# Francis-Rings/MotionEditor

Hardware: AMD Instinct MI355X
Metric: denoise-steps/sec, 24f x 512^2 two-branch UNet3D+ControlNet(+adapter+K/V injection) (higher is better)
Workload: dtype f16

## Files before the change

include/motioned.h:

```cpp
#ifndef MOTIONED_H
#define MOTIONED_H

#include <stdint.h>

#ifdef __cplusplus
extern "C" {
#endif

#define ME_OK 0
#define ME_EINVAL (-1)
#define ME_EHIP (-2)

#define ME_ABI_VERSION 9

int me_abi_version(void);
const char* me_last_error(void);
const char* me_last_kernel(void);
int me_device_info(int* cus, int* lds_bytes, char* arch, int arch_len);

#define ME_GATHER_DENSE 0
#define ME_GATHER_CONV3 1
#define ME_GATHER_TCONV 2

typedef struct me_gemm_args {
// ... 10 lines not shown
  const void* bias;
  const void* rowvec;
  int32_t ldrv, rows_per_vec;
  const void* res;
  int32_t ldr;
  const void* res2;
  int32_t ldr2;
  int32_t geglu;
  int32_t act;
  float alpha;
  int32_t res_rows;
  int32_t res2_rows;
  void* work;
  int64_t work_bytes;
  int32_t splits_;
  int32_t sel_rows;
  void* C2;
  int32_t c2_col0, c2_dh;
  int64_t c2_hs;
  int32_t m_off;
  const void* ln_stats;
  const void* ln_colsum;
  const void* ln_cvec;
  int64_t ln_stride;
  int32_t ln_parts;
  float ln_eps;
  void* ln_out;
  int64_t ln_out_stride;
} me_gemm_args;

int me_gemm(const me_gemm_args* a, void* stream);
int me_ln_stats(const void* X, int32_t ldx, int64_t rows, int32_t C, void* stats, int64_t stride, void* stream);
int64_t me_gemm_work_bytes(const me_gemm_args* a);

typedef struct me_conv_small_args {
  const void* in;
  const void* W;
  const void* bias;
  void* out;
  int32_t n_img, Cin, Cout, H, Wd;
  int64_t img_stride, ch_stride;
  int32_t in_is_f16;
  int32_t silu;
  int32_t frames;
  int64_t frame_stride;
} me_conv_small_args;

int me_conv_small(const me_conv_small_args* a, void* stream);

#define ME_SEG_PLAIN 0
#define ME_SEG_DUAL_CUR 1
#define ME_SEG_DUAL_PREV 2
#define ME_SEG_DUAL_BIN 3

typedef struct me_attn_args {
  const void* Q;
  const void* K;
  const void* V;
  void* O;
  int32_t ldq, ldk, ldv, ldo;
  int32_t heads, dh;
  int32_t n_items, nq, nk, nseg;
  const int32_t* seg_item;
  const int32_t* seg_mode;
  const void* mask;
  float scale;
// ... 199 lines not shown
```

motioneditor_amd/capi.py:

```python
from __future__ import annotations

import ctypes as C
from pathlib import Path

LIB_PATH = Path(__import__("os").environ.get("ME_LIB") or Path(__file__).resolve().parent / "libmotioned.so")

ME_OK, ME_EINVAL, ME_EHIP = 0, -1, -2
ABI_VERSION = 9
GATHER_DENSE, GATHER_CONV3, GATHER_TCONV = 0, 1, 2
SEG_PLAIN, SEG_DUAL_CUR, SEG_DUAL_PREV, SEG_DUAL_BIN = 0, 1, 2, 3

_i32, _i64, _f32, _vp = C.c_int32, C.c_int64, C.c_float, C.c_void_p


class GemmArgs(C.Structure):
    _fields_ = [
        ("X", _vp), ("W", _vp), ("C", _vp),
        ("M", _i32), ("N", _i32), ("K", _i32),
        ("ldx", _i32), ("ldc", _i32), ("gather", _i32),
        ("Hin", _i32), ("Win", _i32), ("Hout", _i32), ("Wout", _i32), ("stride", _i32), ("ups", _i32), ("pad0", _i32),
        ("frames", _i32), ("npix", _i32), ("chunk", _i32),
        ("frame0", _i32), ("frames_total", _i32), ("halo_prev", _i32), ("halo_next", _i32),
        ("bias", _vp), ("rowvec", _vp), ("ldrv", _i32), ("rows_per_vec", _i32),
        ("res", _vp), ("ldr", _i32), ("res2", _vp), ("ldr2", _i32), ("geglu", _i32), ("act", _i32), ("alpha", _f32), ("res_rows", _i32), ("res2_rows", _i32),
# ... 60 lines not shown
        ("q_frames", _i32), ("q_frame0", _i32), ("kv_parts", _i32), ("q_parts", _i32),
    ]


class GroupNormArgs(C.Structure):
    _fields_ = [
        ("X", _vp), ("Y", _vp), ("gamma", _vp), ("beta", _vp), ("stats", _vp),
        ("rows", _i32), ("rows_per_group", _i32),
        ("C", _i32), ("ldx", _i32), ("ldy", _i32), ("groups", _i32), ("eps", _f32), ("silu", _i32),
    ]


class LayerNormArgs(C.Structure):
    _fields_ = [
        ("X", _vp), ("Y", _vp), ("gamma", _vp), ("beta", _vp),
        ("rows", _i32), ("C", _i32), ("ldx", _i32), ("ldy", _i32), ("eps", _f32),
    ]


class PlanStats(C.Structure):
    _fields_ = [("launches", _i64), ("event_records", _i64), ("event_waits", _i64), ("arg_bytes", _i64), ("replays", _i64), ("streams", _i32)]


class PlanNodeInfo(C.Structure):
    _fields_ = [("kind", _i32), ("stream", _i32), ("event", _i32), ("grid", C.c_uint32 * 3), ("block", C.c_uint32 * 3), ("lds_bytes", C.c_uint32),
                ("n_args", _i32), ("arg_bytes", _i64)]


PLAN_LAUNCH, PLAN_RECORD, PLAN_WAIT = 0, 1, 2

SYMBOLS = {
    "me_abi_version": (C.c_int, []),
    "me_gemm_work_bytes": (_i64, [C.POINTER(GemmArgs)]),
    "me_last_error": (C.c_char_p, []),
    "me_last_kernel": (C.c_char_p, []),
    "me_device_info": (C.c_int, [C.POINTER(C.c_int), C.POINTER(C.c_int), C.c_char_p, C.c_int]),
    "me_gemm": (C.c_int, [C.POINTER(GemmArgs), _vp]),
    "me_conv_small": (C.c_int, [C.POINTER(ConvSmallArgs), _vp]),
    "me_attn": (C.c_int, [C.POINTER(AttnArgs), _vp]),
    "me_tattn": (C.c_int, [C.POINTER(TAttnArgs), _vp]),
    "me_groupnorm": (C.c_int, [C.POINTER(GroupNormArgs), _vp]),
    "me_groupnorm_scratch_bytes": (C.c_int64, [_i32, _i32, _i32]),
    "me_groupnorm_stats": (C.c_int, [C.POINTER(GroupNormArgs), _vp]),
    "me_groupnorm_apply": (C.c_int, [C.POINTER(GroupNormArgs), _i64, _vp]),
    "me_layernorm": (C.c_int, [C.POINTER(LayerNormArgs), _vp]),
    "me_ln_stats": (C.c_int, [_vp, _i32, _i64, _i32, _vp, _i64, _vp]),
    "me_softmax_rows": (C.c_int, [_vp, _i32, _vp, _i32, _i64, _i32, _vp]),
    "me_axpy_rows": (C.c_int, [_vp, _i32, _vp, _i32, _vp, _i32, _i64, _i32, _f32, _vp]),
    "me_attn_vsum_bytes": (_i64, [_i32, _i32]),
    "me_attn_fallback_blocks": (_i64, [_i32]),
    "me_geglu_bwd": (C.c_int, [_vp, _i32, _vp, _i32, _vp, _i32, _i64, _i32, _vp]),
    "me_layernorm_bwd": (C.c_int, [_vp, _i32, _vp, _i32, _vp, _vp, _i32, _i64, _i32, C.c_float, _vp]),
    "me_groupnorm_bwd": (C.c_int, [_vp, _i32, _vp, _i32, _vp, _vp, _vp, _i32, _i64, _i32, _i32, _i32, C.c_float, _i32, _vp, _vp]),
    "me_groupnorm_bwd_scratch_bytes": (_i64, [_i32, _i32, _i32]),
    "me_tattn_bwd": (C.c_int, [_vp, _i32, _vp, _i32, _vp, _i32, _vp, _i32, _vp, _i32, _vp, _i32, _vp, _i32, _i32, _i32, _i32, _i32, _i32, C.c_float, _vp]),
    "me_softmax_bwd_rows": (C.c_int, [_vp, _i32, _vp, _i32, _vp, _i32, _i64, _i32, C.c_float, _vp]),
    "me_relu_bwd": (C.c_int, [_vp, _i32, _vp, _i32, _vp, _i32, _i64, _i32, _vp]),
    "me_copy_rows": (C.c_int, [_vp, _i32, _vp, _i32, _i64, _i32, _vp]),
    "me_copy_blocks": (C.c_int, [_vp, _i32, _vp, _i32, _i32, _i32, _i64, _i32, _i64, _i64, _i64, _i64, _vp]),
    "me_silu": (C.c_int, [_vp, _vp, _i64, _vp]),
    "me_relu": (C.c_int, [_vp, _vp, _i64, _vp]),
    "me_timestep_embed": (C.c_int, [_vp, _i32, _i32, _f32, _vp]),
    "me_cfg_ddim": (C.c_int, [_vp, _vp, _vp, _i32, _i32, _i32, _i32, _i32, _f32, _f32, _f32, _vp]),
    "me_timestep_embed_dev": (C.c_int, [_vp, _i32, _i32, _vp, _vp]),
    "me_cfg_ddim_dev": (C.c_int, [_vp, _vp, _vp, _i32, _i32, _i32, _i32, _i32, _vp, _vp]),
    "me_gaussian_sample": (C.c_int, [_vp, _vp, _i32, _vp, _i32, _i32, _f32, _vp]),
# ... 69 lines not shown
```

motioneditor_amd/csrc/gemm.hip:

```cpp
#include "me_common.h"
#include "../../include/motioned.h"
#include <stdio.h>
#include <stdlib.h>

namespace {

constexpr int BK = 64;
#ifndef WIDE_TERMS
#define WIDE_TERMS 0
#endif
constexpr int STAGE_REG = 0, STAGE_GLDS = 1, STAGE_BUF = 2;
constexpr int ROWEPI_FLAG = 1 << 30, TILEORDER_FLAG = 1 << 29;

template <bool NT = false>
__device__ __forceinline__ void st16(f16* p, uint4 v) {
  if constexpr (NT) {
    typedef unsigned u32x4 __attribute__((ext_vector_type(4)));
    __builtin_nontemporal_store((u32x4){v.x, v.y, v.z, v.w}, reinterpret_cast<u32x4*>(p));
  } else {
    *reinterpret_cast<uint4*>(p) = v;
  }
}
template <bool NT = false>
__device__ __forceinline__ void st8(f16* p, uint2 v) {
// ... 43 lines not shown
    const int ky = tap / 3, kx = tap - ky * 3;
    const int iy = r.y0 + ky, ix = r.x0 + kx;
    const int sh = a.ups ? 1 : 0;
    const int Hv = a.Hin << sh, Wv = a.Win << sh;
    if (iy < 0 || iy >= Hv || ix < 0 || ix >= Wv) return -1;
    if (a.ups == 2 && ((iy | ix) & 1)) return -1;
    return r.base + (iy >> sh) * a.Win + (ix >> sh);
  }
  const int dt = tap - 1;
  const int ftot = a.frames_total > 0 ? a.frames_total : a.frames;
  const int gf = a.frame0 + r.y0, gs = gf + dt;
  if (gs < 0 || gs >= ftot || gs / a.chunk != gf / a.chunk) return -1;
  const int ls = r.y0 + dt;
  if (ls >= 0 && ls < a.frames) return r.base + dt * a.npix;
  const int hb = ls < 0 ? a.halo_prev : a.halo_next;
  return hb < 0 ? -1 : hb + r.x0;
}

template <int NT, int MT, int WN>
__device__ __forceinline__ void init_acc(const me_gemm_args& a, f32x4 (&acc)[NT][MT], int n0, int wn, int lane, bool use_bias = true) {
  const f16* __restrict__ bias = use_bias ? reinterpret_cast<const f16*>(a.bias) : nullptr;
  const int nb = n0 + wn * WN + (lane >> 4) * 4;
  const float inv_alpha = bias ? 1.0f / a.alpha : 0.f;
#pragma unroll
  for (int j = 0; j < NT; ++j) {
    U64 b;
    b.u = (bias && nb + 16 * j < a.N) ? *reinterpret_cast<const uint2*>(bias + nb + 16 * j) : make_uint2(0u, 0u);
    const f32x4 v = {(float)b.e[0] * inv_alpha, (float)b.e[1] * inv_alpha, (float)b.e[2] * inv_alpha, (float)b.e[3] * inv_alpha};
#pragma unroll
    for (int i = 0; i < MT; ++i) acc[j][i] = v;
  }
}

template <int NT, int MT>
__device__ __forceinline__ void ln_fold_acc(const me_gemm_args& a, f32x4 (&acc)[NT][MT], int mbase, int nbase, int lane) {
  const float* __restrict__ st = reinterpret_cast<const float*>(a.ln_stats);
  const float* __restrict__ cs = reinterpret_cast<const float*>(a.ln_colsum);
  const float* __restrict__ cv = reinterpret_cast<const float*>(a.ln_cvec);
  const float invK = 1.0f / (float)a.K;
  float nmean[MT], rstd[MT];
#pragma unroll
  for (int i = 0; i < MT; ++i) {
    const int m = min(mbase + i * 16 + (lane & 15), a.M - 1);
    float s1 = 0.f, s2 = 0.f;
    for (int p = 0; p < a.ln_parts; ++p) {
      const f32x2 v = *reinterpret_cast<const f32x2*>(st + (long)p * a.ln_stride + 2 * (long)m);
      s1 += v[0];
      s2 += v[1];
    }
    const float mu = s1 * invK;
    const float var = __builtin_fmaf(-mu, mu, s2 * invK);
    nmean[i] = -mu;
    rstd[i] = rsqrtf(fmaxf(var, 0.f) + a.ln_eps);
  }
#pragma unroll
  for (int j = 0; j < NT; ++j) {
    const int n = nbase + j * 16 + (lane >> 4) * 4;
    f32x4 s = {0.f, 0.f, 0.f, 0.f}, c = {0.f, 0.f, 0.f, 0.f};
    if (n < a.N) {
      s = *reinterpret_cast<const f32x4*>(cs + n);
      c = *reinterpret_cast<const f32x4*>(cv + n);
    }
#pragma unroll
    for (int i = 0; i < MT; ++i)
#pragma unroll
      for (int r = 0; r < 4; ++r) acc[j][i][r] = __builtin_fmaf(rstd[i], __builtin_fmaf(nmean[i], s[r], acc[j][i][r]), c[r]);
  }
}

constexpr int LN_LDS_BYTES = 12288, LN_LDS_COLSUM = 8192, LN_LDS_CVEC = 10240;
template <int NT, int MT>
__device__ __forceinline__ void ln_fold_acc_lds(const me_gemm_args& a, f32x4 (&acc)[NT][MT], const char* img, int rloc, int cloc, int lane) {
  const float invK = 1.0f / (float)a.K;
  uint2 v[MT][4];
#pragma unroll
  for (int i = 0; i < MT; ++i) {
    const int row = rloc + i * 16 + (lane & 15);
#pragma unroll
    for (int p = 0; p < 4; ++p) v[i][p] = *reinterpret_cast<const uint2*>(img + p * 2048 + row * 8);
  }
  float nmean[MT], rstd[MT];
#pragma unroll
  for (int i = 0; i < MT; ++i) {
    float s1 = 0.f, s2 = 0.f;
#pragma unroll
    for (int p = 0; p < 4; ++p) {
      s1 += __uint_as_float(v[i][p].x);
      s2 += __uint_as_float(v[i][p].y);
    }
    const float mu = s1 * invK;
    const float var = __builtin_fmaf(-mu, mu, s2 * invK);
    nmean[i] = -mu;
    rstd[i] = rsqrtf(fmaxf(var, 0.f) + a.ln_eps);
  }
#pragma unroll
  for (int j = 0; j < NT; ++j) {
    const int col = cloc + j * 16 + (lane >> 4) * 4;
    const uint4 su = *reinterpret_cast<const uint4*>(img + LN_LDS_COLSUM + col * 4), cu = *reinterpret_cast<const uint4*>(img + LN_LDS_CVEC + col * 4);
    const f32x4 s = {__uint_as_float(su.x), __uint_as_float(su.y), __uint_as_float(su.z), __uint_as_float(su.w)};
    const f32x4 c = {__uint_as_float(cu.x), __uint_as_float(cu.y), __uint_as_float(cu.z), __uint_as_float(cu.w)};
// ... 1103 lines not shown
    cluster(1, 0, NT0);
    ME_BAR();
  }
  if (wr == 0) ME_BAR();
  asm volatile("s_waitcnt vmcnt(0)" ::: "memory");
#undef ME_BAR
#undef ME_LGKM0

  if constexpr (EPI <= 0) {
    if (a.ln_stats) {
      if constexpr (LN_LDS) ln_fold_acc_lds<NT, MT>(a, acc, smem + 2 * BUFBYTES, wr * GR, wc * WN, lane);
      else ln_fold_acc<NT, MT>(a, acc, m0 + wr * GR, n0 + wc * WN, lane);
    }
  }

  if constexpr (EPI >= 0 && BN == 256) {
    __builtin_amdgcn_s_barrier();
    return epilogue_geglu_rowpass<NT, MT, WN>(a, acc, m0, n0, wr, wc, lane, smem);
  } else if constexpr (EPI >= 0) {
    __builtin_amdgcn_s_barrier();
    char* scr = smem + wave * (32 * (WN * 2 + 16));
    const int mw0 = m0 + wr * GR, nw0 = n0 + wc * WN;
    const LnOutCtx lnx = {m0, wr, wc, tid, smem + 8 * (32 * (WN * 2 + 16))};
    return epilogue_rowpass<EPI, NT, MT, WN>(a, acc, mw0, nw0, lane, scr, lnx);
  } else {
    auto rowfn = [&](int i) {
      const int m = m0 + wr * GR + i * 16 + (lane & 15);
      return m < a.M ? m : -1;
    };
    epilogue<NT, MT, WN>(a, acc, rowfn, m0, n0, wc, lane, nullptr, 0);
  }
}

__global__ __launch_bounds__(256) void gemm_splitk_reduce_kernel(const me_gemm_args a) {
  const int vpr = a.N / 4;
  const long total = (long)a.M * vpr;
  const float* __restrict__ wk = reinterpret_cast<const float*>(a.work);
  const f16* __restrict__ bias = reinterpret_cast<const f16*>(a.bias);
  const f16* __restrict__ rowvec = reinterpret_cast<const f16*>(a.rowvec);
  const f16* res = reinterpret_cast<const f16*>(a.res);
  const f16* res2 = reinterpret_cast<const f16*>(a.res2);
  f16* C = reinterpret_cast<f16*>(a.C);
  const long plane = (long)a.M * a.N;
  for (long idx = (long)blockIdx.x * 256 + threadIdx.x; idx < total; idx += (long)gridDim.x * 256) {
    const int m = (int)(idx / vpr);
    const int n = (int)(idx - (long)m * vpr) * 4;
    f32x4 v = *reinterpret_cast<const f32x4*>(wk + (long)m * a.N + n);
    for (int s_ = 1; s_ < a.splits_; ++s_) v += *reinterpret_cast<const f32x4*>(wk + s_ * plane + (long)m * a.N + n);
    v *= a.alpha;
    if (bias) {
      U64 b;
      b.u = *reinterpret_cast<const uint2*>(bias + n);
#pragma unroll
      for (int r = 0; r < 4; ++r) v[r] += (float)b.e[r];
    }
    U64 rv, r1, r2, o;
    if (rowvec) rv.u = *reinterpret_cast<const uint2*>(rowvec + (long)(m / a.rows_per_vec) * a.ldrv + n);
    if (res) r1.u = *reinterpret_cast<const uint2*>(res + (long)(a.res_rows > 0 ? m % a.res_rows : m) * a.ldr + n);
    if (res2) r2.u = *reinterpret_cast<const uint2*>(res2 + (long)(a.res2_rows > 0 ? m % a.res2_rows : m) * a.ldr2 + n);
    if (a.act == 0) {
#pragma unroll
      for (int r = 0; r < 4; ++r) {
        f16 h = (f16)v[r];
        if (rowvec) h = h + rv.e[r];
        if (res) h = h + r1.e[r];
        if (res2) h = h + r2.e[r];
// ... 271 lines not shown
  const int nit = (a->K / 64) * (a->gather == ME_GATHER_CONV3 ? 9 : (a->gather == ME_GATHER_TCONV ? 3 : 1));
  const long blocks = (long)((a->M + 127) / 128) * ((a->N + 159) / 160);
  const int S = choose_split(a, blocks, nit);
  return S > 1 ? (int64_t)4 * a->M * a->N * 4 : 0;
}

static int gemm_dispatch(const me_gemm_args* a, void* stream);

extern "C" int me_gemm(const me_gemm_args* a, void* stream) {
  if (!a || !a->X || !a->W || !a->C) { me_set_error("me_gemm: null pointer"); return ME_EINVAL; }
  if (a->ln_stats) {
    if (a->gather != ME_GATHER_DENSE || a->bias || a->alpha != 1.0f || a->rowvec || a->res || a->res2 || a->act || !a->ln_colsum || !a->ln_cvec || a->ln_parts < 1 || a->ln_parts > 4 || a->ln_stride < 2 * (int64_t)a->M ||
        (a->ln_stride & 1) || ((uintptr_t)a->ln_stats & 7) || (((uintptr_t)a->ln_colsum | (uintptr_t)a->ln_cvec) & 15) || !(a->ln_eps > 0.f)) {
      me_set_error("me_gemm: a LayerNorm-folded launch is dense, has no bias (it is inside ln_cvec), no rowvec / residual / activation and alpha == 1; ln_colsum / ln_cvec fp32 [N] 16-byte aligned, "
                   "ln_stats 8-byte aligned with 1 <= ln_parts <= 4 parts ln_stride >= 2 M floats apart, ln_eps > 0");
      return ME_EINVAL;
    }
  }
  if (a->ln_out && (a->geglu || a->C2 || a->N % 8 || a->N > 1536 || a->ldc % 8 || ((uintptr_t)a->C & 15) || ((uintptr_t)a->ln_out & 7) || a->ln_out_stride < 2 * (int64_t)a->M || (a->ln_out_stride & 1))) {
    me_set_error("me_gemm: ln_out needs a plain fp16 output of N % 8 == 0, N <= 1536 columns (no GEGLU, no head-major panels), ldc % 8 == 0, and parts >= 2 M floats apart");
    return ME_EINVAL;
  }
  g_ln_fused = false;
  const int rc = gemm_dispatch(a, stream);
  if (rc != ME_OK || !a->ln_out || g_ln_fused) return rc;
  char nm[96];
  snprintf(nm, sizeof(nm), "%s", me_last_kernel());
  const int rc2 = me_ln_stats(reinterpret_cast<const f16*>(a->C) + (long)a->m_off * a->ldc, a->ldc, (int64_t)a->M - a->m_off, a->N,
                              reinterpret_cast<float*>(a->ln_out) + 2 * (long)a->m_off, a->ln_out_stride, stream);
  me_set_kernel(nm);
  return rc2;
}

static int gemm_dispatch(const me_gemm_args* a, void* stream) {
  if (a->M <= 0 || a->N <= 0 || a->K <= 0) { me_set_error("me_gemm: non-positive dimension"); return ME_EINVAL; }
  if (a->K % 8 || a->ldx % 8 || a->ldc % 4 || a->N % 4) { me_set_error("me_gemm: K, ldx must be multiples of 8 and N, ldc of 4"); return ME_EINVAL; }
  if (((uintptr_t)a->X | (uintptr_t)a->W) & 15 || ((uintptr_t)a->C & 7)) { me_set_error("me_gemm: misaligned pointer"); return ME_EINVAL; }
  if (a->gather < 0 || a->gather > 2) { me_set_error("me_gemm: bad gather mode"); return ME_EINVAL; }
  if (a->gather == ME_GATHER_CONV3) {
    if (a->Hin <= 0 || a->Win <= 0 || a->Hout <= 0 || a->Wout <= 0 || (a->stride != 1 && a->stride != 2) || a->ups < 0 || a->ups > 2 ||
        (a->pad0 != 0 && a->pad0 != 1) || a->M % (a->Hout * a->Wout)) { me_set_error("me_gemm: bad conv geometry"); return ME_EINVAL; }
  }
  if (a->gather == ME_GATHER_TCONV) {
    const int ftot = a->frames_total > 0 ? a->frames_total : a->frames;
    if (a->frames <= 0 || a->npix <= 0 || a->chunk <= 0 || ftot % a->chunk || (a->m_off == 0 && a->sel_rows <= a->M && a->M % (a->frames * a->npix)) || a->frame0 < 0 ||
        a->frame0 + a->frames > ftot) { me_set_error("me_gemm: bad tconv geometry"); return ME_EINVAL; }
  }
  if (a->rowvec && (a->rows_per_vec <= 0 || a->ldrv % 4 || ((uintptr_t)a->rowvec & 7))) { me_set_error("me_gemm: bad rowvec"); return ME_EINVAL; }
  if (a->res && (a->ldr % 4 || ((uintptr_t)a->res & 7))) { me_set_error("me_gemm: bad residual"); return ME_EINVAL; }
  if (a->res2 && (a->ldr2 % 4 || ((uintptr_t)a->res2 & 7))) { me_set_error("me_gemm: bad second residual"); return ME_EINVAL; }
  if (a->res_rows < 0 || a->res2_rows < 0) { me_set_error("me_gemm: negative res_rows"); return ME_EINVAL; }
  if (a->act < 0 || a->act > 2) { me_set_error("me_gemm: bad activation"); return ME_EINVAL; }
  if (a->bias && ((uintptr_t)a->bias & 7)) { me_set_error("me_gemm: misaligned bias"); return ME_EINVAL; }
  if (a->geglu && (a->N % 32 || a->rowvec || a->res || a->res2 || a->act || a->alpha != 1.0f)) { me_set_error("me_gemm: geglu needs N % 32 == 0, alpha == 1 and no rowvec/res/act"); return ME_EINVAL; }
  if (a->m_off < 0 || a->m_off >= a->M || (a->m_off > 0 && a->gather == ME_GATHER_CONV3)) { me_set_error("me_gemm: m_off must lie in [0, M) and is for dense / TemporalConv launches"); return ME_EINVAL; }
  if (a->C2 && (a->geglu || a->act || a->rowvec || a->res || a->res2 || a->c2_dh <= 0 || a->c2_dh % 8 || a->c2_col0 < 0 || a->c2_col0 % 16 || a->c2_col0 >= a->N ||
                (a->N - a->c2_col0) % a->c2_dh || a->c2_hs % 8 || a->c2_hs < (int64_t)a->M * a->c2_dh || ((uintptr_t)a->C2 & 15) || a->gather == ME_GATHER_CONV3)) {
    me_set_error("me_gemm: head-major output (C2) needs a term-free epilogue, c2_dh % 8 == 0, c2_col0 % 16 == 0, whole heads, c2_hs % 8 == 0 and >= M * c2_dh, 16-byte alignment");
    return ME_EINVAL;
  }
  hipStream_t st = reinterpret_cast<hipStream_t>(stream);
  const bool wide = a->N % 128 == 0 || a->N % 64 != 0;
  if (stage_impl() == STAGE_GLDS) {
    const int Msel = a->sel_rows > a->M ? a->sel_rows : a->M;
    const long big_blocks = (long)((Msel + 255) / 256) * (a->N / 320);
    if (a->gather == ME_GATHER_CONV3 && a->stride == 1 && a->ups == 0 && !a->pad0 && a->N % 320 == 0 && a->K % 64 == 0 && a->Hin % 16 == 0 &&
// ... 31 lines not shown
```

motioneditor_amd/models/graph.py:

```python
from __future__ import annotations

import contextlib
from dataclasses import dataclass
from typing import Callable, List, Optional, Sequence

import torch

from .. import ops, plan, segments
from ..weights import Packed

HEADS = 8
ADAPTER_CHUNK = 8
HEAD_MAJOR_Q = __import__("os").environ.get("ME_HEAD_MAJOR_Q", "1") != "0"
HEAD_MAJOR_KV = __import__("os").environ.get("ME_HEAD_MAJOR_KV", "1") != "0"
SPLIT_SHARDED_TCONV = __import__("os").environ.get("ME_SPLIT_TCONV", "1") != "0"
INPLACE_SKIPS = __import__("os").environ.get("ME_INPLACE_SKIPS", "1") != "0"
LN_FOLD = __import__("os").environ.get("ME_LN_FOLD", "1") != "0"
COND_EMBED_CACHE = True


@dataclass
class Act:
    t: torch.Tensor
    B: int
    f: int
    h: int
    w: int
    cat: Optional[torch.Tensor] = None

    @property
    def N(self) -> int:
        return self.h * self.w

    @property
    def C(self) -> int:
        return self.t.shape[1]

    def like(self, t: torch.Tensor, h: Optional[int] = None, w: Optional[int] = None) -> "Act":
        return Act(t, self.B, self.f, self.h if h is None else h, self.w if w is None else w)

    def rows_of(self, b: int) -> torch.Tensor:
        n = self.f * self.N
        return self.t[b * n:(b + 1) * n]


@dataclass
class AttnCall:
    q: torch.Tensor
    k: torch.Tensor
    v: torch.Tensor
# ... 81 lines not shown
    return LN_FOLD and not getattr(ops, "recording", False) and getattr(ops, "LN_FOLD", False)


def _gemm_st(*args, **kw):
    if _fold():
        return ops.gemm(*args, ln_out=True, **kw)
    return ops.gemm(*args, **kw), None


class LN:

    def __init__(self, P: Packed, norm: str, x: torch.Tensor, stats: Optional[torch.Tensor] = None):
        self.P, self.norm, self.x, self.stats, self._rows = P, norm, x, stats, None

    def rows(self) -> torch.Tensor:
        if self._rows is None:
            self._rows = ops.layernorm(self.x, self.P.vec(self.norm + ".weight"), self.P.vec(self.norm + ".bias"))
        return self._rows

    def gemm(self, names: Sequence[str], *, geglu_bias: Optional[str] = None, **kw):
        names = list(names)
        geglu = geglu_bias is not None
        if _fold() and self._rows is None:
            if self.stats is None:
                self.stats = ops.ln_stats(self.x)
            w, cs, cv = self.P.ln_fold(self.norm, names, geglu=geglu, bias=geglu_bias)
            return ops.gemm(self.x, w, ln=(self.stats, cs, cv, 1e-5), geglu=geglu, **kw)
        if geglu:
            return ops.gemm(self.rows(), self.P.geglu_mat(names[0]), bias=self.P.geglu_vec(geglu_bias), geglu=True, **kw)
        return ops.gemm(self.rows(), self.P.fused(names) if len(names) > 1 else self.P.mat(names[0]), **kw)


def feed_forward(P: Packed, p: str, n: "LN", res: torch.Tensor, want_stats: bool = False):
    g = n.gemm([p + ".net.0.proj.weight"], geglu_bias=p + ".net.0.proj.bias")
    return (_gemm_st if want_stats else (lambda *a, **k: (ops.gemm(*a, **k), None)))(g, P.mat(p + ".net.2.weight"), bias=P.vec(p + ".net.2.bias"), res=res)


def _ln(P: Packed, p: str, x: torch.Tensor) -> torch.Tensor:
    return ops.layernorm(x, P.vec(p + ".weight"), P.vec(p + ".bias"))


def _qkv(P: Packed, p: str, n: "LN", C: int, shard, B: int = 0, N: int = 0, head_major: bool = False):
    names = [p + ".to_q.weight", p + ".to_k.weight", p + ".to_v.weight"]
    if shard is None:
        if head_major and HEAD_MAJOR_KV and not getattr(ops, "recording", False) and getattr(ops, "HEAD_MAJOR_KV", False):
            if HEAD_MAJOR_Q:
                _, qkv = n.gemm(names, head_major=(0, C // HEADS))
                return qkv[:HEADS], qkv[HEADS:2 * HEADS], qkv[2 * HEADS:]
            q, kv = n.gemm(names, head_major=(C, C // HEADS))
            return q, kv[:HEADS], kv[HEADS:]
        qkv = n.gemm(names)
        return qkv[:, :C], qkv[:, C:2 * C], qkv[:, 2 * C:]
    ext, loc = shard.kv_buffer(n.x.shape[0], 2 * C, B, N, n.x)
    n.gemm(names[1:], out=loc)
    pending = shard.start_kv(ext, B, N, ops.copy_rows)
    q = n.gemm(names[:1])
    kv = shard.finish_kv(pending)
    return q, kv[:, :C], kv[:, C:]


def _temporal_attn(P: Packed, p: str, n: "LN", C: int, B: int, f: int, N: int, dh: int, shard, editor=None, place: str = "") -> torch.Tensor:
    def go(tc):
        return editor(call=tc, is_cross=False, place_in_unet=place, num_heads=HEADS) if editor is not None else tc.run()
    if shard is not None and shard.pixel_sharded(N):
        r = shard.to_pixel_shards(n.rows(), B * f, N, ops.copy_blocks)
        qkv = ops.gemm(r, P.fused([p + ".to_q.weight", p + ".to_k.weight", p + ".to_v.weight"]))
# ... 462 lines not shown
```

motioneditor_amd/ops.py:

```python
from __future__ import annotations

import ctypes as C
from typing import Optional, Sequence, Tuple

import os

import torch

from . import capi
from .capi import AttnArgs, AttnBwdArgs, ConvSmallArgs, GemmArgs, GemmDwArgs, GroupNormArgs, LayerNormArgs, TAttnArgs

F16 = torch.float16


_raw_stream = getattr(torch._C, "_cuda_getCurrentRawStream", None)
_cur_device = getattr(torch._C, "_cuda_getDevice", None)


def _stream() -> int:
    if _raw_stream is not None and _cur_device is not None:
        return _raw_stream(_cur_device())
    return torch.cuda.current_stream().cuda_stream


# ... 83 lines not shown
        if col0 == 0:
            out = panels.view(-1)[:8 * M].view(M, 8)
    if out is None:
        if row_range is not None:
            raise ValueError("gemm: row_range writes into a caller-provided `out` of all M rows")
        out = empty(M, n_out, x)
    _chk2d(out, "gemm.out")
    if out.shape[0] < M or out.shape[1] < n_out:
        raise ValueError("gemm: out too small")
    a.X, a.W, a.C = x.data_ptr(), w.data_ptr(), out.data_ptr()
    a.M, a.N, a.K = M, N, K
    if row_range is not None:
        lo, hi = row_range
        if not (0 <= lo < hi <= M) or conv is not None:
            raise ValueError("gemm: row_range must lie inside [0, M) (dense / TemporalConv launches)")
        a.m_off, a.M = lo, hi
        a.sel_rows = max(a.sel_rows, M)
    a.ldx, a.ldc = x.stride(0), out.stride(0)
    a.bias = _p(bias)
    if rowvec is not None:
        _chk2d(rowvec, "gemm.rowvec")
        a.rowvec, a.ldrv, a.rows_per_vec = rowvec.data_ptr(), rowvec.stride(0), rows_per_vec
    if res is not None:
        _chk2d(res, "gemm.res")
        a.res, a.ldr = res.data_ptr(), res.stride(0)
    if res2 is not None:
        _chk2d(res2, "gemm.res2")
        a.res2, a.ldr2 = res2.data_ptr(), res2.stride(0)
    a.geglu = 1 if geglu else 0
    a.act = act
    a.alpha = alpha
    a.res_rows, a.res2_rows = res_rows, res2_rows
    if ln is not None:
        st_, cs_, cv_, eps_ = ln
        if st_.dtype != torch.float32 or st_.dim() != 3 or st_.shape[2] != 2 or st_.stride(2) != 1 or st_.stride(1) != 2 or st_.shape[1] < M \
                or cs_.dtype != torch.float32 or cv_.dtype != torch.float32 or cs_.numel() != N or cv_.numel() != N or not cs_.is_contiguous() or not cv_.is_contiguous():
            raise ValueError("gemm: ln = (fp32 stats [parts, rows, 2], fp32 colsum [N], fp32 cvec [N], eps)")
        a.ln_stats, a.ln_colsum, a.ln_cvec, a.ln_eps = st_.data_ptr(), cs_.data_ptr(), cv_.data_ptr(), eps_
        a.ln_parts, a.ln_stride = st_.shape[0], st_.stride(0)
    so = None
    if ln_out:
        if panels is not None or geglu:
            raise ValueError("gemm: ln_out is for plain row outputs")
        so = torch.empty((n_out // 320 if n_out % 320 == 0 else 1, M, 2), dtype=torch.float32, device=x.device)
        a.ln_out, a.ln_out_stride = so.data_ptr(), so.stride(0)
    if SELECT_ROWS_SCALE > 1:
        a.sel_rows = M * SELECT_ROWS_SCALE
    for r_, n_ in ((res, res_rows), (res2, res2_rows)):
        if r_ is not None and r_.shape[0] < (n_ or M):
            raise ValueError("gemm: residual has fewer rows than the output reads")
    if N >= 1280 and M <= 8192:
        nb = capi.lib().me_gemm_work_bytes(C.byref(a))
        if nb > 0:
            a.work, a.work_bytes = _work(nb, x.device, "splitk").data_ptr(), nb
    e0 = _pb()
    capi.check(capi.lib().me_gemm(C.byref(a), _stream()), "me_gemm")
    if e0 is not None:
        rows_in = (M // (conv[2] * conv[3])) * conv[0] * conv[1] if conv is not None else M
        n_terms = (res is not None) + (res2 is not None)
        n_hm = panels.numel() // M if panels is not None else 0
        _pe(e0, "gemm", 2.0 * M * N * K * taps, 2.0 * (rows_in * K + N * K * taps + M * n_out * (1 + n_terms) + M * n_hm), f"M{M} N{N} K{K} taps{taps}{' geglu' if geglu else ''}{' +b' if bias is not None else ''}{' +rv' if rowvec is not None else ''}"
            f"{' +res' if res is not None else ''}{' +res2' if res2 is not None else ''}{' act' + str(act) if act else ''}{' a' + str(alpha) if alpha != 1.0 else ''}{' ln' if ln is not None else ''}{' lnout' if ln_out else ''}", _last_kernel())
    if panels is not None and n_out == 0:
        return None, panels
    out = out[:M, :n_out] if (out.shape[0] != M or out.shape[1] != n_out) else out
    if so is not None:
        return out, so
    return out if panels is None else (out, panels)


def ln_stats(x: torch.Tensor) -> torch.Tensor:
    _chk2d(x, "ln_stats.x")
    rows, Cc = x.shape
    st = torch.empty((Cc // 320 if Cc % 320 == 0 else 1, rows, 2), dtype=torch.float32, device=x.device)
    e0 = _pb()
    capi.check(capi.lib().me_ln_stats(x.data_ptr(), x.stride(0), rows, Cc, st.data_ptr(), st.stride(0), _stream()), "me_ln_stats")
    _pe(e0, "layernorm", 3.0 * rows * Cc, 2.0 * rows * Cc, "stats", "ln_stats")
    return st


def gemm_splits_k(M: int, N: int, K: int, taps: int = 1) -> bool:
    if not (N >= 1280 and M <= 8192):
        return False
    a = GemmArgs()
    a.M, a.N, a.K = M, N, K
    a.gather = capi.GATHER_TCONV if taps == 3 else (capi.GATHER_CONV3 if taps == 9 else capi.GATHER_DENSE)
    return capi.lib().me_gemm_work_bytes(C.byref(a)) > 0


def conv_small(inp: torch.Tensor, w: torch.Tensor, bias: Optional[torch.Tensor], *, n_img: int, Cin: int, H: int, Wd: int,
               img_stride: int, ch_stride: int, frames: int = 0, frame_stride: int = 0, silu: bool = False) -> torch.Tensor:
    if w.dtype != torch.float32 or (bias is not None and bias.dtype != torch.float32):
        raise ValueError("conv_small: weights and bias must be fp32")
    Cout = w.shape[0]
    out = torch.empty((n_img * H * Wd, Cout), dtype=F16, device=inp.device)
    a = ConvSmallArgs()
    a.inp, a.W, a.bias, a.out = inp.data_ptr(), w.data_ptr(), _p(bias), out.data_ptr()
    a.n_img, a.Cin, a.Cout, a.H, a.Wd = n_img, Cin, Cout, H, Wd
    a.img_stride, a.ch_stride = img_stride, ch_stride
    if inp.dtype == torch.float32:
        a.in_is_f16 = 0
# ... 601 lines not shown
```

Before: 6.733.

## Fuse LayerNorm-folded GEGLU FF1 and FF2 into one FFN kernel for C=320

Adds an ffn_kernel that, for each 128-row block, computes the LN-folded GEGLU projection in 128-column hidden slices. Each slice is kept in LDS and immediately multiplied into the FF2 accumulator with bias, residual and optional LN-stats epilogue. This avoids writing and re-reading the M x 1280 hidden activation to global memory and drops one launch per feed-forward at width 320. In exchange it uses one 512-thread block per CU with large LDS and streams weights repeatedly per block, so grid parallelism and weight traffic change.

```diff
diff --git a/include/motioned.h b/include/motioned.h
--- a/include/motioned.h
+++ b/include/motioned.h
@@ -66,6 +66,7 @@
 int me_gemm(const me_gemm_args* a, void* stream);
 int me_ln_stats(const void* X, int32_t ldx, int64_t rows, int32_t C, void* stats, int64_t stride, void* stream);
 int64_t me_gemm_work_bytes(const me_gemm_args* a);
+int me_ffn(const me_gemm_args* ff1, const me_gemm_args* ff2, void* stream);
 
 typedef struct me_conv_small_args {
   const void* in;
diff --git a/motioneditor_amd/capi.py b/motioneditor_amd/capi.py
--- a/motioneditor_amd/capi.py
+++ b/motioneditor_amd/capi.py
@@ -116,6 +116,7 @@
 SYMBOLS = {
     "me_abi_version": (C.c_int, []),
     "me_gemm_work_bytes": (_i64, [C.POINTER(GemmArgs)]),
+    "me_ffn": (C.c_int, [C.POINTER(GemmArgs), C.POINTER(GemmArgs), _vp]),
     "me_last_error": (C.c_char_p, []),
     "me_last_kernel": (C.c_char_p, []),
     "me_device_info": (C.c_int, [C.POINTER(C.c_int), C.POINTER(C.c_int), C.c_char_p, C.c_int]),
diff --git a/motioneditor_amd/csrc/gemm.hip b/motioneditor_amd/csrc/gemm.hip
--- a/motioneditor_amd/csrc/gemm.hip
+++ b/motioneditor_amd/csrc/gemm.hip
@@ -99,13 +99,10 @@
   }
 }
 
-template <int NT, int MT>
-__device__ __forceinline__ void ln_fold_acc(const me_gemm_args& a, f32x4 (&acc)[NT][MT], int mbase, int nbase, int lane) {
+template <int MT>
+__device__ __forceinline__ void ln_row_stats(const me_gemm_args& a, float (&nmean)[MT], float (&rstd)[MT], int mbase, int lane) {
   const float* __restrict__ st = reinterpret_cast<const float*>(a.ln_stats);
-  const float* __restrict__ cs = reinterpret_cast<const float*>(a.ln_colsum);
-  const float* __restrict__ cv = reinterpret_cast<const float*>(a.ln_cvec);
   const float invK = 1.0f / (float)a.K;
-  float nmean[MT], rstd[MT];
 #pragma unroll
   for (int i = 0; i < MT; ++i) {
     const int m = min(mbase + i * 16 + (lane & 15), a.M - 1);
@@ -120,6 +117,11 @@
     nmean[i] = -mu;
     rstd[i] = rsqrtf(fmaxf(var, 0.f) + a.ln_eps);
   }
+}
+template <int NT, int MT>
+__device__ __forceinline__ void ln_fold_cols(const me_gemm_args& a, f32x4 (&acc)[NT][MT], const float (&nmean)[MT], const float (&rstd)[MT], int nbase, int lane) {
+  const float* __restrict__ cs = reinterpret_cast<const float*>(a.ln_colsum);
+  const float* __restrict__ cv = reinterpret_cast<const float*>(a.ln_cvec);
 #pragma unroll
   for (int j = 0; j < NT; ++j) {
     const int n = nbase + j * 16 + (lane >> 4) * 4;
@@ -133,6 +135,12 @@
 #pragma unroll
       for (int r = 0; r < 4; ++r) acc[j][i][r] = __builtin_fmaf(rstd[i], __builtin_fmaf(nmean[i], s[r], acc[j][i][r]), c[r]);
   }
+}
+template <int NT, int MT>
+__device__ __forceinline__ void ln_fold_acc(const me_gemm_args& a, f32x4 (&acc)[NT][MT], int mbase, int nbase, int lane) {
+  float nmean[MT], rstd[MT];
+  ln_row_stats<MT>(a, nmean, rstd, mbase, lane);
+  ln_fold_cols<NT, MT>(a, acc, nmean, rstd, nbase, lane);
 }
 
 constexpr int LN_LDS_BYTES = 12288, LN_LDS_COLSUM = 8192, LN_LDS_CVEC = 10240;
@@ -1302,6 +1310,134 @@
   }
 }
 
+constexpr int FFN_C = 320, FFN_H = 4 * FFN_C, FFN_BM = 128;
+constexpr int FFN_W1 = 5 * FFN_BM * 128, FFN_W2 = FFN_W1 + 2 * FFN_BM * 128, FFN_LDS = FFN_W2 + FFN_C * 128;
+__global__ __launch_bounds__(512, 1) void ffn_kernel(const me_gemm_args a1, const me_gemm_args a2) {
+  constexpr int KT1 = FFN_C / BK, NS = FFN_H / BK, MT = 4, NT1 = 2, NT2 = 5, WN2 = FFN_C / 4, TILE = FFN_BM * 128;
+  static_assert(FFN_LDS <= 160 * 1024 && KT1 * 8 == FFN_C / 8, "LDS budget; one W2 piece per wave and ff1 K tile");
+  extern __shared__ __attribute__((aligned(16))) char smem[];
+  const int tid = threadIdx.x, lane = tid & 63;
+  const int wave = __builtin_amdgcn_readfirstlane(tid >> 6);
+  const int wr = wave >> 2, wc = wave & 3;
+  const int m0 = blockIdx.x * FFN_BM;
+
+  typedef __attribute__((address_space(3))) void* lptr_t;
+  constexpr unsigned OOB = 0x80000000u;
+  const auto xsrd = __builtin_amdgcn_make_buffer_rsrc(const_cast<void*>(static_cast<const void*>(reinterpret_cast<const f16*>(a1.X) + (long)m0 * a1.ldx)), 0, OOB, 0x00020000);
+  const auto w1srd = __builtin_amdgcn_make_buffer_rsrc(const_cast<void*>(a1.W), 0, (unsigned)(2 * FFN_H * FFN_C * 2), 0x00020000);
+  const auto w2srd = __builtin_amdgcn_make_buffer_rsrc(const_cast<void*>(a2.W), 0, (unsigned)(FFN_C * FFN_H * 2), 0x00020000);
+  const int prow = lane >> 3;
+  const int scol = ((lane & 7) ^ ((4 * (wave & 1) + (lane >> 4)) & 7)) * 8;
+
+#pragma unroll
+  for (int i = 0; i < 10; ++i) {
+    const int p = wave + 8 * i, kt = p >> 4, r = (p & 15) * 8;
+    const unsigned off = m0 + r + prow < a1.M ? (unsigned)(((long)(r + prow) * a1.ldx + kt * BK + scol) * 2) : OOB;
+    __builtin_amdgcn_raw_ptr_buffer_load_lds(xsrd, (lptr_t)(smem + kt * TILE + r * 128), 16, (int)off, 0, 0, 0);
+  }
+  unsigned w1o[2];
+#pragma unroll
+  for (int i = 0; i < 2; ++i) w1o[i] = (unsigned)(((8 * (wave + 8 * i) + prow) * FFN_C + scol) * 2);
+  const unsigned w2o = (unsigned)(((8 * wave + prow) * FFN_H + scol) * 2);
+  auto issue_w1 = [&](int s, int kc, int buf) {
+    const int so = __builtin_amdgcn_readfirstlane((s * FFN_BM * FFN_C + kc * BK) * 2);
+#pragma unroll
+    for (int i = 0; i < 2; ++i)
+      __builtin_amdgcn_raw_ptr_buffer_load_lds(w1srd, (lptr_t)(smem + FFN_W1 + buf * TILE + 8 * (wave + 8 * i) * 128), 16, (int)w1o[i], so, 0, 0);
+  };
+  auto issue_w2 = [&](int s, int kc) {
+    const int so = __builtin_amdgcn_readfirstlane(s * BK * 2 + kc * 64 * FFN_H * 2);
+    __builtin_amdgcn_raw_ptr_buffer_load_lds(w2srd, (lptr_t)(smem + FFN_W2 + 8 * (wave + 8 * kc) * 128), 16, (int)w2o, so, 0, 0);
+  };
+  issue_w1(0, 0, 0);
+
+  f32x4 acc2[NT2][MT];
+  init_acc<NT2, MT, WN2>(a2, acc2, 0, wc, lane);
+  float nmean[MT], rstd[MT];
+  ln_row_stats<MT>(a1, nmean, rstd, m0 + wr * 64, lane);
+
+  const int frow = lane & 15, fg = lane >> 4;
+  const int c0 = (fg ^ ((frow >> 1) & 7)) << 4;
+  const int lx = (wr * 64 + frow) * 128 + c0;
+  const int lw1 = (wc * 32 + frow) * 128 + c0;
+  const int lw2 = (wc * WN2 + frow) * 128 + c0;
+  char* const hid = smem + FFN_W1 + TILE;
+#define FFN_STEP_END()                                 \
+  do {                                                 \
+    __builtin_amdgcn_sched_barrier(0);                 \
+    asm volatile("s_waitcnt vmcnt(0)" ::: "memory");   \
+    __builtin_amdgcn_sched_barrier(0);                 \
+    __builtin_amdgcn_s_barrier();                      \
+    asm volatile("" ::: "memory");                     \
+    __builtin_amdgcn_sched_barrier(0);                 \
+  } while (0)
+  FFN_STEP_END();
+
+  for (int s = 0; s < NS; ++s) {
+    f32x4 acc1[NT1][MT];
+#pragma unroll
+    for (int j = 0; j < NT1; ++j)
+#pragma unroll
+      for (int i = 0; i < MT; ++i) acc1[j][i] = f32x4{0.f, 0.f, 0.f, 0.f};
+#pragma unroll
+    for (int kc = 0; kc < KT1; ++kc) {
+      if (kc + 1 < KT1) issue_w1(s, kc + 1, (kc + 1) & 1);
+      issue_w2(s, kc);
+      const char* wb = smem + FFN_W1 + (kc & 1) * TILE;
+      const char* xb = smem + kc * TILE;
+      f16x8 fw[2][NT1], fx[2][MT];
+#pragma unroll
+      for (int ks = 0; ks < 2; ++ks) {
+#pragma unroll
+        for (int j = 0; j < NT1; ++j) fw[ks][j] = *reinterpret_cast<const f16x8*>(wb + (lw1 ^ (64 * ks)) + j * 2048);
+#pragma unroll
+        for (int i = 0; i < MT; ++i) fx[ks][i] = *reinterpret_cast<const f16x8*>(xb + (lx ^ (64 * ks)) + i * 2048);
+      }
+#pragma unroll
+      for (int ks = 0; ks < 2; ++ks)
+#pragma unroll
+        for (int j = 0; j < NT1; ++j)
+#pragma unroll
+          for (int i = 0; i < MT; ++i) acc1[j][i] = mfma16(fw[ks][j], fx[ks][i], acc1[j][i]);
+      FFN_STEP_END();
+    }
+    ln_fold_cols<NT1, MT>(a1, acc1, nmean, rstd, s * FFN_BM + wc * 32, lane);
+#pragma unroll
+    for (int i = 0; i < MT; ++i) {
+      const f32x2 v01 = geglu2(f32x2{acc1[0][i][0], acc1[0][i][1]}, f32x2{acc1[1][i][0], acc1[1][i][1]});
+      const f32x2 v23 = geglu2(f32x2{acc1[0][i][2], acc1[0][i][3]}, f32x2{acc1[1][i][2], acc1[1][i][3]});
+      union { f16x2 h[2]; uint2 u; } o;
+      o.h[0] = __builtin_convertvector(v01, f16x2);
+      o.h[1] = __builtin_convertvector(v23, f16x2);
+      const int row = wr * 64 + i * 16 + frow;
+      *reinterpret_cast<uint2*>(hid + row * 128 + (((2 * wc + (fg >> 1)) ^ ((row >> 1) & 7)) << 4) + (fg & 1) * 8) = o.u;
+    }
+    __syncthreads();
+    if (s + 1 < NS) issue_w1(s + 1, 0, 0);
+    {
+      f16x8 fw[2][NT2], fh[2][MT];
+#pragma unroll
+      for (int ks = 0; ks < 2; ++ks) {
+#pragma unroll
+        for (int j = 0; j < NT2; ++j) fw[ks][j] = *reinterpret_cast<const f16x8*>(smem + FFN_W2 + (lw2 ^ (64 * ks)) + j * 2048);
+#pragma unroll
+        for (int i = 0; i < MT; ++i) fh[ks][i] = *reinterpret_cast<const f16x8*>(hid + (lx ^ (64 * ks)) + i * 2048);
+      }
+#pragma unroll
+      for (int ks = 0; ks < 2; ++ks)
+#pragma unroll
+        for (int j = 0; j < NT2; ++j)
+#pragma unroll
+          for (int i = 0; i < MT; ++i) acc2[j][i] = mfma16(fw[ks][j], fh[ks][i], acc2[j][i]);
+    }
+    FFN_STEP_END();
+  }
+#undef FFN_STEP_END
+  char* scr = smem + wave * (32 * (WN2 * 2 + 16));
+  const LnOutCtx lnx = {m0, wr, wc, tid, smem + 8 * (32 * (WN2 * 2 + 16))};
+  epilogue_rowpass<4, NT2, MT, WN2>(a2, acc2, m0 + wr * 64, wc * WN2, lane, scr, lnx);
+}
+
 __global__ __launch_bounds__(256) void gemm_splitk_reduce_kernel(const me_gemm_args a) {
   const int vpr = a.N / 4;
   const long total = (long)a.M * vpr;
@@ -1639,6 +1775,49 @@
   return rc2;
 }
 
+extern "C" int me_ffn(const me_gemm_args* f1, const me_gemm_args* f2, void* stream) {
+  if (!f1 || !f2 || !f1->X || !f1->W || !f2->W || !f2->C || !f2->res) { me_set_error("me_ffn: null pointer"); return ME_EINVAL; }
+  const int64_t M = f1->M;
+  if (M <= 0 || f2->M != M || f1->m_off || f2->m_off || f1->K != FFN_C || f1->N != 2 * FFN_H || f2->K != FFN_H || f2->N != FFN_C) {
+    me_set_error("me_ffn: ff1 is [M, 320] x [2560, 320]^T, ff2 [M, 1280] x [320, 1280]^T, both over the same M rows from row 0");
+    return ME_EINVAL;
+  }
+  if (f1->gather != ME_GATHER_DENSE || !f1->geglu || f1->bias || f1->alpha != 1.0f || f1->rowvec || f1->res || f1->res2 || f1->act || f1->C2 || f1->ln_out ||
+      f1->ldx % 8 || f1->ldx < FFN_C || (((uintptr_t)f1->X | (uintptr_t)f1->W) & 15) ||
+      !f1->ln_stats || !f1->ln_colsum || !f1->ln_cvec || f1->ln_parts < 1 || f1->ln_parts > 4 || f1->ln_stride < 2 * M || (f1->ln_stride & 1) ||
+      ((uintptr_t)f1->ln_stats & 7) || (((uintptr_t)f1->ln_colsum | (uintptr_t)f1->ln_cvec) & 15) || !(f1->ln_eps > 0.f)) {
+    me_set_error("me_ffn: ff1 is a dense LayerNorm-folded GEGLU launch (no bias: it is inside ln_cvec; no terms, alpha == 1), X / W 16-byte aligned with ldx % 8 == 0, "
+                 "ln_colsum / ln_cvec fp32 16-byte aligned, ln_stats 8-byte aligned with 1 <= ln_parts <= 4 parts ln_stride >= 2 M floats apart, ln_eps > 0");
+    return ME_EINVAL;
+  }
+  if (f2->gather != ME_GATHER_DENSE || f2->geglu || f2->ln_stats || f2->alpha != 1.0f || f2->rowvec || f2->res2 || f2->act || f2->C2 || f2->res_rows < 0 ||
+      f2->ldc % 8 || f2->ldc < FFN_C || f2->ldr % 8 || (((uintptr_t)f2->W | (uintptr_t)f2->C | (uintptr_t)f2->res) & 15) || ((uintptr_t)f2->bias & 7) ||
+      (f2->ln_out && (((uintptr_t)f2->ln_out & 7) || f2->ln_out_stride < 2 * M || (f2->ln_out_stride & 1)))) {
+    me_set_error("me_ffn: ff2 is a dense launch with bias and residual only (alpha == 1), W / C / res 16-byte aligned with ldc, ldr % 8 == 0, bias 8-byte aligned, "
+                 "ln_out 8-byte aligned with parts >= 2 M floats apart");
+    return ME_EINVAL;
+  }
+  static bool attr_set_dev[64] = {};
+  int dev_id = 0;
+  (void)hipGetDevice(&dev_id);
+  bool& attr_set = attr_set_dev[dev_id & 63];
+  if (!attr_set) {
+    if (hipFuncSetAttribute(reinterpret_cast<const void*>(&ffn_kernel), hipFuncAttributeMaxDynamicSharedMemorySize, FFN_LDS) != hipSuccess) {
+      me_set_error("me_ffn: hipFuncSetAttribute(MaxDynamicSharedMemorySize) failed");
+      return ME_EHIP;
+    }
+    attr_set = true;
+  }
+  (void)hipGetLastError();
+  hipLaunchKernelGGL(ffn_kernel, dim3((unsigned)((M + FFN_BM - 1) / FFN_BM)), dim3(512), FFN_LDS, reinterpret_cast<hipStream_t>(stream), *f1, *f2);
+  me_set_kernel("ffn_kernel");
+  if (hipGetLastError() != hipSuccess) {
+    me_set_error("me_ffn: kernel launch failed");
+    return ME_EHIP;
+  }
+  return ME_OK;
+}
+
 static int gemm_dispatch(const me_gemm_args* a, void* stream) {
   if (a->M <= 0 || a->N <= 0 || a->K <= 0) { me_set_error("me_gemm: non-positive dimension"); return ME_EINVAL; }
   if (a->K % 8 || a->ldx % 8 || a->ldc % 4 || a->N % 4) { me_set_error("me_gemm: K, ldx must be multiples of 8 and N, ldc of 4"); return ME_EINVAL; }
diff --git a/motioneditor_amd/models/graph.py b/motioneditor_amd/models/graph.py
--- a/motioneditor_amd/models/graph.py
+++ b/motioneditor_amd/models/graph.py
@@ -16,6 +16,7 @@
 SPLIT_SHARDED_TCONV = __import__("os").environ.get("ME_SPLIT_TCONV", "1") != "0"
 INPLACE_SKIPS = __import__("os").environ.get("ME_INPLACE_SKIPS", "1") != "0"
 LN_FOLD = __import__("os").environ.get("ME_LN_FOLD", "1") != "0"
+FFN_FUSED = __import__("os").environ.get("ME_FFN_FUSED", "1") != "0"
 COND_EMBED_CACHE = True
 
 
@@ -163,6 +164,12 @@
 
 
 def feed_forward(P: Packed, p: str, n: "LN", res: torch.Tensor, want_stats: bool = False):
+    ffn = getattr(ops, "ffn", None) if FFN_FUSED and _fold() and n._rows is None else None
+    if ffn is not None and n.x.shape[1] in ops.FFN_WIDTHS:
+        if n.stats is None:
+            n.stats = ops.ln_stats(n.x)
+        w1, cs, cv = P.ln_fold(n.norm, [p + ".net.0.proj.weight"], geglu=True, bias=p + ".net.0.proj.bias")
+        return ffn(n.x, w1, (n.stats, cs, cv, 1e-5), P.mat(p + ".net.2.weight"), bias=P.vec(p + ".net.2.bias"), res=res, ln_out=want_stats)
     g = n.gemm([p + ".net.0.proj.weight"], geglu_bias=p + ".net.0.proj.bias")
     return (_gemm_st if want_stats else (lambda *a, **k: (ops.gemm(*a, **k), None)))(g, P.mat(p + ".net.2.weight"), bias=P.vec(p + ".net.2.bias"), res=res)
 
diff --git a/motioneditor_amd/ops.py b/motioneditor_amd/ops.py
--- a/motioneditor_amd/ops.py
+++ b/motioneditor_amd/ops.py
@@ -139,18 +139,12 @@
     a.alpha = alpha
     a.res_rows, a.res2_rows = res_rows, res2_rows
     if ln is not None:
-        st_, cs_, cv_, eps_ = ln
-        if st_.dtype != torch.float32 or st_.dim() != 3 or st_.shape[2] != 2 or st_.stride(2) != 1 or st_.stride(1) != 2 or st_.shape[1] < M \
-                or cs_.dtype != torch.float32 or cv_.dtype != torch.float32 or cs_.numel() != N or cv_.numel() != N or not cs_.is_contiguous() or not cv_.is_contiguous():
-            raise ValueError("gemm: ln = (fp32 stats [parts, rows, 2], fp32 colsum [N], fp32 cvec [N], eps)")
-        a.ln_stats, a.ln_colsum, a.ln_cvec, a.ln_eps = st_.data_ptr(), cs_.data_ptr(), cv_.data_ptr(), eps_
-        a.ln_parts, a.ln_stride = st_.shape[0], st_.stride(0)
+        _set_ln(a, ln, M, N, "gemm")
     so = None
     if ln_out:
         if panels is not None or geglu:
             raise ValueError("gemm: ln_out is for plain row outputs")
-        so = torch.empty((n_out // 320 if n_out % 320 == 0 else 1, M, 2), dtype=torch.float32, device=x.device)
-        a.ln_out, a.ln_out_stride = so.data_ptr(), so.stride(0)
+        so = _set_ln_out(a, M, n_out, x.device)
     if SELECT_ROWS_SCALE > 1:
         a.sel_rows = M * SELECT_ROWS_SCALE
     for r_, n_ in ((res, res_rows), (res2, res2_rows)):
@@ -174,6 +168,54 @@
     if so is not None:
         return out, so
     return out if panels is None else (out, panels)
+
+
+def _set_ln(a: GemmArgs, ln, M: int, N: int, what: str) -> None:
+    st_, cs_, cv_, eps_ = ln
+    if st_.dtype != torch.float32 or st_.dim() != 3 or st_.shape[2] != 2 or st_.stride(2) != 1 or st_.stride(1) != 2 or st_.shape[1] < M \
+            or cs_.dtype != torch.float32 or cv_.dtype != torch.float32 or cs_.numel() != N or cv_.numel() != N or not cs_.is_contiguous() or not cv_.is_contiguous():
+        raise ValueError(f"{what}: ln = (fp32 stats [parts, rows, 2], fp32 colsum [N], fp32 cvec [N], eps)")
+    a.ln_stats, a.ln_colsum, a.ln_cvec, a.ln_eps = st_.data_ptr(), cs_.data_ptr(), cv_.data_ptr(), eps_
+    a.ln_parts, a.ln_stride = st_.shape[0], st_.stride(0)
+
+
+def _set_ln_out(a: GemmArgs, M: int, n_out: int, device) -> torch.Tensor:
+    so = torch.empty((n_out // 320 if n_out % 320 == 0 else 1, M, 2), dtype=torch.float32, device=device)
+    a.ln_out, a.ln_out_stride = so.data_ptr(), so.stride(0)
+    return so
+
+
+FFN_WIDTHS = (320,)
+
+
+def ffn(x: torch.Tensor, w1: torch.Tensor, ln: Tuple[torch.Tensor, torch.Tensor, torch.Tensor, float], w2: torch.Tensor, *,
+        bias: torch.Tensor, res: torch.Tensor, ln_out: bool = False):
+    _chk2d(x, "ffn.x")
+    _chk2d(res, "ffn.res")
+    for w, nm in ((w1, "w1"), (w2, "w2")):
+        if w.dtype != F16 or not w.is_contiguous() or w.dim() != 3 or w.shape[1] != 1:
+            raise ValueError(f"ffn.{nm}: expected contiguous fp16 [N, 1, K]")
+    M = x.shape[0]
+    if res.shape[0] < M:
+        raise ValueError("ffn: residual has fewer rows than the output")
+    a1, a2 = GemmArgs(), GemmArgs()
+    a1.gather = a2.gather = capi.GATHER_DENSE
+    a1.X, a1.W, a1.ldx = x.data_ptr(), w1.data_ptr(), x.stride(0)
+    a1.M, a1.N, a1.K = M, w1.shape[0], w1.shape[2]
+    a1.geglu, a1.alpha = 1, 1.0
+    _set_ln(a1, ln, M, w1.shape[0], "ffn")
+    out = empty(M, w2.shape[0], x)
+    a2.W, a2.C, a2.ldc = w2.data_ptr(), out.data_ptr(), out.stride(0)
+    a2.M, a2.N, a2.K = M, w2.shape[0], w2.shape[2]
+    a2.bias, a2.alpha = _p(bias), 1.0
+    a2.res, a2.ldr = res.data_ptr(), res.stride(0)
+    so = _set_ln_out(a2, M, w2.shape[0], x.device) if ln_out else None
+    e0 = _pb()
+    capi.check(capi.lib().me_ffn(C.byref(a1), C.byref(a2), _stream()), "me_ffn")
+    if e0 is not None:
+        N1, N2, K1 = w1.shape[0], w2.shape[0], w1.shape[2]
+        _pe(e0, "gemm", 2.0 * M * (N1 * K1 + N2 * w2.shape[2]), 2.0 * (M * K1 + N1 * K1 + N2 * w2.shape[2] + 2 * M * N2), f"M{M} ffn C{K1}{' lnout' if ln_out else ''}", _last_kernel())
+    return out, so
 
 
 def ln_stats(x: torch.Tensor) -> torch.Tensor:
```

After: 6.748, median of 6. Within noise of the previous version (+0.2%).
